# Sara-H-dev/Semantic_Segmentation_Of_StyleGAN2_Artifacts

Hardware: AMD Instinct MI355X
Metric: training images/sec at 1024^2 bs=8 per GPU (MS-UNet Swin-T, fwd+DynamicLoss+bwd+AdamW) (higher is better)
Workload: dtype bf16; 1 GPU; 1xMI355X 1024x1024 bs=8 Swin-T MS-UNet train step; model=MS-UNet swin_t, global_batch=8, world_size=1, img_size=1024, parallelism=dp1, grad_allreduce=f32, dead_branches=executed (no grad), step_execution=eager, params=42881040

## Files before the change

include/msunet_hip.h:

```cpp
#ifndef MSUNET_HIP_H
#define MSUNET_HIP_H

#ifdef __cplusplus
extern "C" {
#endif

int msu_layernorm_fwd(int dtype, int mode, const void* x, const void* b, const float* bscale,
                      long rows_per_sample, void* s_out, const float* gamma, const float* beta,
                      void* y, float* mean, float* rstd, long rows, int C, int H, int W, int Cin,
                      float eps, void* stream);
int msu_layernorm_bwd(int dtype, int mode, const void* dy, const void* x, const void* dres,
                      const float* gamma, const float* mean, const float* rstd, void* dx,
                      void* db, const float* bscale, long rows_per_sample, float* part,
                      int nparts, float* dgamma, float* dbeta, long rows, int C, int H, int W,
                      int Cin, int accumulate, void* stream);
int msu_layernorm_bwd3(int dtype, int mode, const void* dy, const void* x, const void* dres,
                       const void* dres2, const void* dres3, const float* gamma, const float* mean,
                       const float* rstd, void* dx, void* db, const float* bscale, long rows_per_sample,
                       float* part, int nparts, float* dgamma, float* dbeta, long rows, int C, int H, int W,
                       int Cin, int accumulate, void* stream);
int msu_ln_part_blocks(long rows, int C);
int msu_colsum_batch(int nseg, const float* const* part, const long* stride, const int* nparts, const int* n,
                     float* const* out, int accumulate, void* stream);
int msu_tail_reduce_mode(int mode);
// ... 48 lines not shown
                      float* workspace, void* unused, int nchunk, int B, int H, int W, int Cin,
                      int Cout, void* stream);
int msu_conv3x3_wgrad2(int dtype, int in_mode, const void* X, const void* dY, float* dW, float* db,
                       float* workspace, int nchunk, int B, int H, int W, int Cin, int Cout, int accumulate,
                       void* stream);

int msu_win_attn_qkv_supported(int C, int nh);
int msu_win_attn_qkv_fwd(int dtype, const void* x, const void* w_qkv, const float* b_qkv, const float* table,
                         void* out, void* qkv_out, void* keep, float* workspace, int B, int H, int W, int C, int nh,
                         int shift, float p_drop, unsigned long long seed, const unsigned long long* seed_dev,
                         void* stream);
int msu_win_attn_qkv_fwd2(int dtype, const void* x, const void* w_qkv, const float* b_qkv, const float* table,
                          const void* w_proj, const float* b_proj, void* out, void* o_out, void* qkv_out, void* keep,
                          float* workspace, int B, int H, int W, int C, int nh, int shift, float p_drop,
                          unsigned long long seed, const unsigned long long* seed_dev, void* stream);

int msu_wgrad_splits(long M, int N, int K);
long msu_wgrad_workspace(long M, int N, int K);
int msu_linear_wgrad(int dtype, const void* dY, const void* X, float* dW, float* db, float* workspace,
                     long M, int N, int K, int accumulate, void* stream);
int msu_linear_wgrad_ld(int dtype, const void* dY, const void* X, float* dW, long ldw, float* db,
                        float* workspace, long M, int N, int K, int accumulate, void* stream);
int msu_linear_wgrad_plan(int dtype, long M, int N, int K, int* out6);

int msu_linear_bwd_supported(long M, int K, int N);
long msu_linear_bwd_workspace(long M, int K, int N);
int msu_linear_bwd(int dtype, const void* dY, const void* X, const void* Wt, const void* H, void* dX, float* dW,
                   float* db, float* workspace, long M, int K, int N, int accumulate, void* stream);

int msu_tok_gemm_supported(long M, int N, int K);
int msu_tok_gemm_supported_epi(long M, int N, int K, int epi);
int msu_tok_gemm(int dtype, const void* A, const void* A2, int K1, const void* W, const float* bias, void* Y,
                 void* Y2, const void* H, long M, int N, int K, int epi, void* stream);
int msu_tok_gemm_plan(long M, int N, int K, long* out6);
int msu_tok_gemm_plan_epi(long M, int N, int K, int epi, int concat, long* out6);
int msu_nt_gemm_supported(long M, int N, int K);
int msu_nt_gemm_plan(long M, int N);
int msu_nt_gemm_plan2(long M, int N, int K, int epi, int wkn, long* out8);
int msu_nt_gemm_mode(int mode);
int msu_nt_gemm(int dtype, const void* A, const void* W, const float* bias, void* Y, void* Y2, const void* H,
                long M, int N, int K, int epi, void* stream);
int msu_nt_gemm_cat(int dtype, const void* A, const void* A2, int K1, const void* W, const float* bias, void* Y,
                    long M, int N, int K, void* stream);
int msu_nt_gemm_kn(int dtype, const void* A, const void* Wk, const float* bias, void* Y, void* Y2, const void* H,
                   long M, int N, int K, int epi, void* stream);

// ... 82 lines not shown
```

semantic_segmentation_of_stylegan2_artifacts_amd/_lib.py:

```python
import ctypes
import os

from . import switches

_HERE = os.path.dirname(os.path.abspath(__file__))
LIB_PATH = switches.get("MSU_LIB_OVERRIDE") or os.path.join(_HERE, "libmsunet_hip.so")

P = ctypes.c_void_p
I = ctypes.c_int
L = ctypes.c_long
F = ctypes.c_float
D = ctypes.c_double
U64 = ctypes.c_ulonglong

SIGNATURES = {
    "msu_ln_part_blocks": (I, [L, I]),
    "msu_layernorm_fwd": (I, [I, I, P, P, P, L, P, P, P, P, P, P, L, I, I, I, I, F, P]),
    "msu_layernorm_bwd": (I, [I, I, P, P, P, P, P, P, P, P, P, L, P, I, P, P, L, I, I, I, I, I, P]),
    "msu_layernorm_bwd3": (I, [I, I, P, P, P, P, P, P, P, P, P, P, P, L, P, I, P, P, L, I, I, I, I, I, P]),
    "msu_reduce_rows": (I, [P, I, I, L, P, I, P]),
    "msu_tail_reduce_mode": (I, [I]),
    "msu_conv_mode": (I, [I]),
    "msu_conv3x3_route": (I, [I, I, I]),
    "msu_head_fwd": (I, [I, P, P, P, P, P, P, P, L, I, F, P]),
# ... 31 lines not shown
    "msu_grad_sumsq2": (I, [P, L, P, L, P, I, P, P]),
    "msu_grad_clip_scale": (I, [P, I, P, D, P, P, P]),
    "msu_adamw_dev": (I, [P, P, P, P, L, P, D, D, D, D, P, P, P]),
    "msu_adamw_dev2": (I, [P, P, P, P, L, P, D, D, D, D, P, P, P, I, I, P]),
    "msu_adamw_dev3": (I, [P, P, P, P, P, L, P, D, D, D, D, D, P, P, P, I, I, P]),
    "msu_swap_cast": (I, [P, P, P, I, L, P]),
    "msu_step_advance": (I, [P, P, P]),
    "msu_loss_scale_step": (I, [P, P, P, P, P, P, D, D, I, P]),
    "msu_cast": (I, [I, P, P, L, P]),
    "msu_colsum_batch": (I, [I, P, P, P, P, P, I, P]),
    "msu_conv3x3_weight": (I, [I, P, P, I, I, I, P]),
    "msu_transpose16_multi": (I, [P, P, P, I, I, P]),
    "msu_conv3x3_fwd": (I, [I, I, P, P, P, P, I, I, I, I, I, P]),
    "msu_conv3x3_fwd2": (I, [I, I, P, P, P, P, P, I, I, I, I, I, P]),
    "msu_conv3x3_dgrad": (I, [I, I, P, P, P, P, I, I, I, I, I, P]),
    "msu_conv3x3_wgrad_workspace": (L, [I, I, I, I, I]),
    "msu_conv3x3_wgrad": (I, [I, I, P, P, P, P, P, P, I, I, I, I, I, I, P]),
    "msu_conv3x3_wgrad2": (I, [I, I, P, P, P, P, P, I, I, I, I, I, I, I, P]),
    "msu_wgrad_splits": (I, [L, I, I]),
    "msu_wgrad_workspace": (L, [L, I, I]),
    "msu_linear_wgrad": (I, [I, P, P, P, P, P, L, I, I, I, P]),
    "msu_linear_wgrad_ld": (I, [I, P, P, P, L, P, P, L, I, I, I, P]),
    "msu_linear_wgrad_plan": (I, [I, L, I, I, P]),
    "msu_linear_bwd_supported": (I, [L, I, I]),
    "msu_linear_bwd_workspace": (L, [L, I, I]),
    "msu_linear_bwd": (I, [I, P, P, P, P, P, P, P, P, L, I, I, I, P]),
    "msu_tok_gemm_supported": (I, [L, I, I]),
    "msu_tok_gemm_supported_epi": (I, [L, I, I, I]),
    "msu_tok_gemm": (I, [I, P, P, I, P, P, P, P, P, L, I, I, I, P]),
    "msu_tok_gemm_plan": (I, [L, I, I, P]),
    "msu_tok_gemm_plan_epi": (I, [L, I, I, I, I, P]),
    "msu_nt_gemm_supported": (I, [L, I, I]),
    "msu_nt_gemm_plan": (I, [L, I]),
    "msu_nt_gemm_plan2": (I, [L, I, I, I, I, P]),
    "msu_nt_gemm_mode": (I, [I]),
    "msu_nt_gemm": (I, [I, P, P, P, P, P, P, L, I, I, I, P]),
    "msu_nt_gemm_kn": (I, [I, P, P, P, P, P, P, L, I, I, I, P]),
    "msu_nt_gemm_cat": (I, [I, P, P, I, P, P, P, L, I, I, P]),
    "msu_metrics_nblk": (I, [L]),
    "msu_seg_metrics": (I, [I, P, P, I, L, F, P, I, P, P]),
    "msu_augment_batch": (I, [P, P, P, P, P, P, I, I, I, P]),
    "msu_augment_gather": (I, [P, P, P, I, P, P, P, P, I, I, I, P]),
    "msu_pred_maps_nblk": (I, [I, I]),
    "msu_pred_maps": (I, [I, P, P, P, I, I, I, F, F, F, F, I, I, P, P, P, P, P, P, P, P]),
}

# ... 38 lines not shown
```

semantic_segmentation_of_stylegan2_artifacts_amd/csrc/gemm_wgrad.hip:

```cpp
#include <stdlib.h>

#include "common.h"
#include "mfma_frag.h"
#include "reduce.h"

#ifndef MSU_EXP
#define MSU_EXP 0
#endif

namespace {

constexpr int BM = 64;

MSU_DEV void unpack8(const u32x4& q, float (&v)[8]) {
#pragma unroll
  for (int i = 0; i < 4; ++i) {
    v[2 * i] = __uint_as_float(q[i] << 16);
    v[2 * i + 1] = __uint_as_float(q[i] & 0xffff0000u);
  }
}

template <typename T, int NTW>
__global__ void __launch_bounds__(256) wgrad_kernel(const T* __restrict__ dY, const T* __restrict__ X,
                                                    float* __restrict__ part, float* __restrict__ dbpart,
// ... 69 lines not shown
      for (int r = 0; r < BM; ++r) dbacc += to_f32(A[r * LDT + tid]);
    }
    if (more) store_regs(buf ^ 1);
    __syncthreads();
    buf ^= 1;
  }
  float* out = part + (long)blockIdx.y * N * K;
#pragma unroll
  for (int i = 0; i < NTW; ++i)
#pragma unroll
    for (int j = 0; j < NTW; ++j)
#pragma unroll
      for (int r = 0; r < 4; ++r) {
        const int n = n0 + wn + 16 * i + (lane >> 4) * 4 + r;
        const int k = k0 + wk + 16 * j + (lane & 15);
        if (n < N && k < K) out[(long)n * K + k] = acc[i][j][r];
      }
  if (do_bias && tid < BT && n0 + tid < N) dbpart[(long)blockIdx.y * N + n0 + tid] = dbacc;
}

template <int WN, int WK> constexpr int wgrad_nw() { return WN * WK == 3 ? 3 : 4; }

template <typename T, int NTW, int WN, int WK, int NST>
__global__ void __launch_bounds__(256) wgrad_wave_kernel(const bf16_t* __restrict__ dY, const bf16_t* __restrict__ X,
                                                         float* __restrict__ part, float* __restrict__ dbpart,
                                                         long M, int N, int K, long mchunk, int ntiles) {
  constexpr int NW = wgrad_nw<WN, WK>();
  constexpr int WM = NW / (WN * WK), WT = 16 * NTW, BN = WN * WT, BK = WK * WT, RS = 32 * WM;
  static_assert(WM * WN * WK == NW, "wave split");
  constexpr int SA = (BN + 8) / 8, SB = (BK + 8) / 8;
  constexpr int LA = 8 * SA, LB = 8 * SB;
  constexpr int SLOTS = RS * (SA + SB);
  constexpr int INS = ((SLOTS + 63) / 64 + NW - 1) / NW * NW;
  constexpr int PER_WAVE = INS / NW;
  constexpr int STG = INS * 64 * 8;
  static_assert(NST >= 2 && PER_WAVE * (NST - 2) < 64, "vmcnt");
  extern __shared__ __attribute__((aligned(16))) unsigned char smem_raw[];
  bf16_t* lds = reinterpret_cast<bf16_t*>(smem_raw);
  const int tid = threadIdx.x, lane = tid & 63;
  const int wave = __builtin_amdgcn_readfirstlane(tid >> 6);
  const int wni = wave % WN, wki = (wave / WN) % WK, wmi = wave / (WN * WK);
  const int ntk = K / BK;
  const int item = xcd_remap(blockIdx.x, gridDim.x);
  const int split = item / ntiles, tile = item - split * ntiles;
  const int tn = tile / ntk, tk = tile - (tile / ntk) * ntk;
  const int n0 = tn * BN, k0 = tk * BK;
  const long m_begin = (long)split * mchunk;
  long m_end = m_begin + mchunk;
  if (m_end > M) m_end = M;
  const int nstage = m_end > m_begin ? (int)((m_end - m_begin + RS - 1) / RS) : 0;

  int srow[PER_WAVE], soff[PER_WAVE];
  bool sisA[PER_WAVE];
#pragma unroll
  for (int r = 0; r < PER_WAVE; ++r) {
    const int s = 64 * (wave + NW * r) + lane;
    if (s < RS * SA) {
      const int row = s / SA, c = s - (s / SA) * SA;
      srow[r] = row;
      soff[r] = row * N + n0 + (c < SA - 1 ? 8 * c : 0);
      sisA[r] = true;
    } else {
      const int t = s < SLOTS ? s - RS * SA : 0;
      const int row = t / SB, c = t - (t / SB) * SB;
      srow[r] = s < SLOTS ? row : RS;
      soff[r] = row * K + k0 + (c < SB - 1 ? 8 * c : 0);
      sisA[r] = false;
    }
  }
  auto issue = [&](int st) __attribute__((always_inline)) {
    bf16_t* buf = lds + (st % NST) * STG;
    const long m0 = m_begin + (long)st * RS;
    const long rem = m_end - m0;
    const int valid = rem > RS ? RS : (rem < 0 ? 0 : (int)rem);
    const bf16_t* baseA = dY + m0 * N;
    const bf16_t* baseB = X + m0 * K;
#pragma unroll
    for (int r = 0; r < PER_WAVE; ++r) {
      const bf16_t* src = (sisA[r] ? baseA : baseB) + soff[r];
      glds16(srow[r] < valid ? (const void*)src : zero_src(64 * r + lane), buf + 64 * 8 * (wave + NW * r));
    }
  };

  f32x4 acc[NTW][NTW];
  f32x4 accb[NTW];
#pragma unroll
  for (int i = 0; i < NTW; ++i) {
    accb[i] = f32x4{0.f, 0.f, 0.f, 0.f};
#pragma unroll
    for (int j = 0; j < NTW; ++j) acc[i][j] = f32x4{0.f, 0.f, 0.f, 0.f};
  }
  const bool do_bias = dbpart != nullptr && tk == 0 && wki == 0;
  const bf16x8 ones = splat8<T>(1.0f, 1.0f, 1.0f);
  const int q = (lane & 15) >> 2, p4 = 4 * (lane & 3), r0 = wmi * 32 + 2 * (4 * ((lane >> 4) & 1) + q) + (lane >> 5);
  const int laneA = r0 * LA + wni * WT + p4, laneB = RS * LA + r0 * LB + wki * WT + p4;
  auto tr8 = [](const bf16_t* p, int second) {
    typedef __attribute__((address_space(3))) msu_v4s lds_v4s;
    const msu_v4s lo = __builtin_amdgcn_ds_read_tr16_b64_v4i16((lds_v4s*)(p));
    const msu_v4s hi = __builtin_amdgcn_ds_read_tr16_b64_v4i16((lds_v4s*)(p + second));
    msu_v4s both[2] = {lo, hi};
    return *reinterpret_cast<bf16x8*>(both);
  };

#pragma unroll
  for (int st = 0; st < NST - 1; ++st) issue(st);
  for (int st = 0; st < nstage; ++st) {
    wait_vmcnt<PER_WAVE * (NST - 2)>();
    __builtin_amdgcn_s_barrier();
    issue(st + NST - 1);
    if constexpr (MSU_EXP & 2) continue;
    const bf16_t* buf = lds + (st % NST) * STG;
    const uint32_t pa = lds_u32(buf + laneA), pb = lds_u32(buf + laneB);
    bf16x8 bf[NTW], af[2];
    unroll_for<NTW>([&](auto J) {
      constexpr int j = decltype(J)::value;
// ... 44 lines not shown
#pragma unroll
          for (int r = 0; r < 4; ++r) mine[(IH * NTW * 4 + (i - h0) * 4 + r) * 64 + lane] = accb[i][r];
        }
      }
      __syncthreads();
      if (wmi == 0) {
#pragma unroll
        for (int w = 1; w < WM; ++w) {
          const float* other = red + ((long)wnk * (WM - 1) + w - 1) * PW;
#pragma unroll
          for (int i = h0; i < h0 + IH; ++i) {
#pragma unroll
            for (int j = 0; j < NTW; ++j)
#pragma unroll
              for (int r = 0; r < 4; ++r) acc[i][j][r] += other[(((i - h0) * NTW + j) * 4 + r) * 64 + lane];
#pragma unroll
            for (int r = 0; r < 4; ++r) accb[i][r] += other[(IH * NTW * 4 + (i - h0) * 4 + r) * 64 + lane];
          }
        }
      }
    });
  }
  if (wmi != 0) return;
  float* out = part + (long)split * N * K;
#pragma unroll
  for (int i = 0; i < NTW; ++i)
#pragma unroll
    for (int j = 0; j < NTW; ++j)
#pragma unroll
      for (int r = 0; r < 4; ++r) {
        const int n = n0 + wni * WT + 16 * i + (lane >> 4) * 4 + r;
        const int k = k0 + wki * WT + 16 * j + (lane & 15);
        out[(long)n * K + k] = acc[i][j][r];
      }
  if (do_bias && (lane & 15) == 0) {
#pragma unroll
    for (int i = 0; i < NTW; ++i)
#pragma unroll
      for (int r = 0; r < 4; ++r)
        dbpart[(long)split * N + n0 + wni * WT + 16 * i + (lane >> 4) * 4 + r] = accb[i][r];
  }
}

struct WavePlan {
  int ntw = 0, wn = 1, wk = 1, nst = 3, S = 1;
  int slabs() const { return S; }
};

inline void pick_wave_split(int nt, int kt, int& wn, int& wk) {
  static const int cand[8][2] = {{4, 1}, {2, 2}, {1, 4}, {3, 1}, {1, 3}, {2, 1}, {1, 2}, {1, 1}};
  long best = -1;
  for (const auto& c : cand) {
    if (nt % c[0] || kt % c[1]) continue;
    const long cost = (long)nt * kt / c[1] + (long)kt * nt / c[0];
    if (best < 0 || cost < best) {
      best = cost;
      wn = c[0];
      wk = c[1];
    }
  }
}

inline WavePlan wave_plan(long M, int N, int K) {
  WavePlan p;
// ... 64 lines not shown
    launch_wave<T, NTW, WN, WK, 3>(grid, dY, X, part, dbpart, M, N, K, mchunk, ntiles, st);                         \
    return 0;                                                                                                       \
  }
  MSU_WAVE(6, 1, 1) MSU_WAVE(6, 2, 1) MSU_WAVE(6, 4, 1) MSU_WAVE(6, 1, 2) MSU_WAVE(6, 2, 2) MSU_WAVE(6, 1, 4)
  MSU_WAVE(6, 3, 1) MSU_WAVE(6, 1, 3)
  MSU_WAVE(8, 1, 1) MSU_WAVE(8, 2, 1) MSU_WAVE(8, 4, 1) MSU_WAVE(8, 1, 2) MSU_WAVE(8, 2, 2) MSU_WAVE(8, 1, 4)
  MSU_WAVE(8, 3, 1) MSU_WAVE(8, 1, 3)
#undef MSU_WAVE
  return -3;
}

inline int tile_of(int N, int K) { return (N % 128 == 0 && K % 128 == 0) ? 128 : 96; }

inline int pick_splits(long M, int N, int K) {
  const int bt = tile_of(N, K);
  const long tiles = (long)((N + bt - 1) / bt) * ((K + bt - 1) / bt);
  long s = (1024 + tiles - 1) / tiles;
  const long max_s = (M + 511) / 512;
  if (s > max_s) s = max_s;
  if (s < 1) s = 1;
  return (int)s;
}

}

extern "C" {

int msu_wgrad_splits(long M, int N, int K) { return pick_splits(M, N, K); }

long msu_wgrad_workspace(long M, int N, int K) {
  const int S = pick_splits(M, N, K);
  long ws = (long)S * N * K + (long)S * N;
  const WavePlan p = wave_plan(M, N, K);
  if (p.ntw) {
    const long w2 = (long)p.slabs() * N * K + (long)p.slabs() * N;
    if (w2 > ws) ws = w2;
  }
  return ws;
}

int msu_linear_wgrad_ld(int dtype, const void* dY, const void* X, float* dW, long ldw, float* db,
                        float* workspace, long M, int N, int K, int accumulate, void* stream) {
  if (N % 8 || K % 8 || M < 0 || ldw < K) return -2;
  hipStream_t st = (hipStream_t)stream;
  if constexpr ((MSU_EXP & 256) != 0) return 0;
  if (M == 0) {
    if (!accumulate) hipMemset2DAsync(dW, sizeof(float) * ldw, 0, sizeof(float) * K, N, st);
    if (db && !accumulate) hipMemsetAsync(db, 0, sizeof(float) * N, st);
    return MSU_CHECK_LAUNCH();
// ... 54 lines not shown
```

semantic_segmentation_of_stylegan2_artifacts_amd/csrc/reduce.h:

```cpp
#pragma once
#include <mutex>

#include "common.h"

extern int g_msu_tail_on;

namespace {

struct ColSegs {
  const float* part[3];
  float* out[3];
  long n[3];
  long stride[3];
  long rowlen[3], ldo[3];
  int bend[3];
  int nseg;
};

template <int PL, int V>
__global__ void __launch_bounds__(256) colsum_kernel(ColSegs sg, int nparts, int accmask) {
  constexpr int NC = 256 / PL;
  typedef float vec __attribute__((ext_vector_type(V)));
  __shared__ vec red[PL][NC + (V == 1 ? 1 : 0)];
  int seg = 0;
// ... 113 lines not shown
#pragma unroll
      for (int u = 0; u < 4; ++u) v[u] = *reinterpret_cast<const float4*>(part + (long)(q + u * CB_PL) * stride + i);
#pragma unroll
      for (int u = 0; u < 4; ++u) { s.x += v[u].x; s.y += v[u].y; s.z += v[u].z; s.w += v[u].w; }
    }
    for (; q < np; q += CB_PL) {
      const float4 v = *reinterpret_cast<const float4*>(part + (long)q * stride + i);
      s.x += v.x; s.y += v.y; s.z += v.z; s.w += v.w;
    }
  }
  __shared__ float4 red[CB_PL][CB_NC];
  red[ly][lx] = s;
  __syncthreads();
  if (ly == 0 && i < n) {
    float4 t = red[0][lx];
#pragma unroll
    for (int k = 1; k < CB_PL; ++k) { t.x += red[k][lx].x; t.y += red[k][lx].y; t.z += red[k][lx].z; t.w += red[k][lx].w; }
    float4* o = reinterpret_cast<float4*>(cb.out[seg] + i);
    if (cb.accumulate) { const float4 v = *o; t.x += v.x; t.y += v.y; t.z += v.z; t.w += v.w; }
    *o = t;
  }
}

constexpr int TAIL_GS = 32, TAIL_SLOTS = 64, TAIL_WORDS = 2048;
__device__ int g_tail_cnt[TAIL_SLOTS * TAIL_WORDS];

inline int tail_slot(hipStream_t st) {
  static std::mutex mu;
  static hipStream_t owner[TAIL_SLOTS];
  static int used = 0;
  if (!g_msu_tail_on) return -1;
  std::lock_guard<std::mutex> lk(mu);
  for (int i = 0; i < used; ++i)
    if (owner[i] == st) return i;
  if (used == TAIL_SLOTS) return -1;
  owner[used] = st;
  return used++;
}

MSU_DEV void tail_st(float* p, float v) { __hip_atomic_store(p, v, __ATOMIC_RELAXED, __HIP_MEMORY_SCOPE_AGENT); }
MSU_DEV void tail_st4(float* p, float4 v) {
  tail_st(p, v.x);
  tail_st(p + 1, v.y);
  tail_st(p + 2, v.z);
  tail_st(p + 3, v.w);
}
// ... 58 lines not shown
```

semantic_segmentation_of_stylegan2_artifacts_amd/ops.py:

```python
import contextlib
import ctypes
import functools

import torch

from . import _lib, switches

_DT = {torch.float32: 0, torch.bfloat16: 1, torch.float16: 2}
_LOW = (torch.bfloat16, torch.float16)


def _dt(t):
    try:
        return _DT[t.dtype]
    except KeyError:
        raise TypeError(f"unsupported activation dtype {t.dtype} (float32 / bfloat16 / float16)") from None


def _need_cuda(*ts):
    for t in ts:
        if t is not None and not t.is_cuda:
            raise RuntimeError("msunet HIP ops need tensors on a HIP device (no CPU fallback)")


# ... 72 lines not shown

def join_side_streams():
    for idx, st in _side_streams.items():
        torch.cuda.current_stream(idx).wait_stream(st)


def _guard_side_write(p, ev):
    p = getattr(p, "_msu_param", p)
    p._msu_side_event = ev
    _side_event_params.append(p)
    if not getattr(p, "_msu_side_hooked", False):
        def hook(grad, p=p):
            e = getattr(p, "_msu_side_event", None)
            if grad is not None and e is not None:
                torch.cuda.current_stream(p.device).wait_event(e)
            return grad
        p.register_hook(hook)
        p._msu_side_hooked = True


_side_keep = []
_side_event_params = []
_ln_pending = []
_bwd_task = -1
backward_discards = 0


_RES_HANDOFF = switches.on("MSU_RES_HANDOFF")
_res_handoff = {}
_res_closed = set()
_res_keys = iter(range(1, 1 << 62))
res_handoff_calls = 0
res_parked = 0
res_dropped = 0


def residual_handoff_key():
    return next(_res_keys) if (_RES_HANDOFF and torch.is_grad_enabled()) else 0


def _park(key, g):
    global res_parked
    if not key:
        return False
    _join_at_end_of_backward()
    if key in _res_closed:
        return False
    _res_handoff.setdefault(key, []).append(g)
    res_parked += 1
    return True


def _take(key):
    if not key:
        return []
    _join_at_end_of_backward()
    _res_closed.add(key)
    return _res_handoff.pop(key, [])


def reset_backward_state():
    global _bwd_task
    _ln_pending.clear()
    _res_handoff.clear()
    _res_closed.clear()
    _side_keep.clear()
    for p in _side_event_params:
        p._msu_side_event = None
    _side_event_params.clear()
    _bwd_task = -1


def _end_of_backward():
    global res_dropped
    _flush_ln()
    res_dropped += sum(len(v) for v in _res_handoff.values())
    join_side_streams()
    reset_backward_state()


def _join_at_end_of_backward():
    global _bwd_task, backward_discards
    task = torch._C._current_graph_task_id()
    if task == _bwd_task and task != -1:
        return
    if _bwd_task != -1:
        backward_discards += 1
        reset_backward_state()
    torch.autograd.Variable._execution_engine.queue_callback(_end_of_backward)
    _bwd_task = task


@contextlib.contextmanager
def _on_side(device, reads=(), writes=()):
    side = _side_stream_for(device)
    side.wait_stream(torch.cuda.current_stream(device))
    _join_at_end_of_backward()
    for t in reads:
        t.record_stream(side)
        _side_keep.append(t)
    with torch.cuda.stream(side):
        yield
    ev = torch.cuda.Event()
    ev.record(side)
    for p in writes:
        if p is not None:
            _guard_side_write(p, ev)
    _notify(*writes)


def _direct(*params):
    return all(p is not None and getattr(p, "_msu_direct", False) and p.grad is not None for p in params)


def _notify(*params):
    if _grad_ready is not None:
        for p in params:
# ... 338 lines not shown
    ctx.bias_param = qkv_bias if isinstance(qkv_bias, torch.nn.Parameter) else None
    ctx.table_param = table if isinstance(table, torch.nn.Parameter) else None
    ctx.cfg = (num_heads, shift, float(p_drop), seed)


def _attn_backward(ctx, dout, _dkeep, _dws=None):
    qkv, qkv_bias, table, seed_dev, keep = ctx.saved_tensors
    if dout is None:
        return None, None, None, None, None, None, None, None
    kp = _p(keep) if keep.numel() else None
    nh, shift, p_drop, seed = ctx.cfg
    B, H, W, C3 = qkv.shape
    C = C3 // 3
    dout = _as(dout, qkv.dtype)
    need = _attn_bwd_ws(qkv.dtype, B, H, W, C, nh)
    ws = getattr(ctx, "aux_ws", None)
    if ws is not None and _ATTN_AUX and qkv.dtype in _LOW and ws.numel() >= need:
        tbl = None
    else:
        ws = torch.empty(need, device=qkv.device, dtype=torch.float32)
        tbl = _p(table)
    dqkv = torch.empty_like(qkv)
    bp, tp = ctx.bias_param, ctx.table_param
    if bp is not None and tp is not None and _side_enabled and _side_attn_tail and _direct(bp, tp):
        _lib.call("msu_win_attn_bwd2", _dt(qkv), _p(qkv), _p(qkv_bias), tbl, _p(dout), _p(dqkv),
                  None, None, _p(ws), B, H, W, C, nh, shift, p_drop, seed, _p(seed_dev), kp,
                  _s(qkv), -1)
        with _on_side(qkv.device, reads=(ws,), writes=(bp, tp)):
            _lib.call("msu_win_attn_bwd_tail2", _dt(qkv), _p(ws), _p(tp.grad), _p(bp.grad), B, H, W, C, nh, 1,
                      _s(qkv))
        return dqkv, None, None, None, None, None, None, None
    dtable = torch.empty_like(table)
    dbias = torch.empty(3 * C, device=qkv.device, dtype=torch.float32)
    _lib.call("msu_win_attn_bwd", _dt(qkv), _p(qkv), _p(qkv_bias), tbl, _p(dout), _p(dqkv),
              _p(dtable), _p(dbias), _p(ws), B, H, W, C, nh, shift, p_drop, seed, _p(seed_dev), kp, _s(qkv))
    return dqkv, dbias, dtable, None, None, None, None, None


_window_attention = _define(
    "window_attention",
    "(Tensor qkv, Tensor qkv_bias, Tensor table, int num_heads, int shift, float p_drop, int seed, Tensor? seed_dev)"
    " -> (Tensor, Tensor, Tensor)",
    _attn_impl, _attn_fake, _attn_setup, _attn_backward)


def window_attention(qkv, qkv_bias, table, num_heads, shift, p_drop=0.0, seed=0, seed_dev=None):
# ... 193 lines not shown
def _gemm_dx(dy, w, epi=TOK_PLAIN, h=None, param=None):
    N, K = w.shape
    M = dy.numel() // N
    wt = _shadow_t(param, w.dtype)
    if gemm_route(M, K, N, epi) == "nt" and wt is None:
        return nt_gemm_kn(dy, w, epi, h)
    return _gemm(dy, _wt(w) if wt is None else wt, None, epi, h)


def _gelu16(h):
    g = torch.empty_like(h)
    _lib.call("msu_gelu_fwd", _dt(h), _p(h), _p(g), h.numel(), _s(h))
    return g


def _wgrad_launch(dy, x, dw, db, M, N, K, acc, x_gelu_of=None):
    if x is None:
        x = _gelu16(x_gelu_of)
    ws = torch.empty(_lib.lib().msu_wgrad_workspace(M, N, K), device=x.device, dtype=torch.float32)
    _lib.call("msu_linear_wgrad_ld", _dt(x), _p(dy), _p(x), _p(dw), dw.stride(0), _p(db), _p(ws), M, N, K, acc,
              _s(x))


def _wgrad(dy, x, weight, bias, M, N, K, x_gelu_of=None, side_ok=True):
    src = x if x is not None else x_gelu_of
    if not (_direct(weight) and (bias is None or _direct(bias))):
        dw = torch.empty(N, K, device=src.device, dtype=torch.float32)
        db = torch.empty(N, device=src.device, dtype=torch.float32) if bias is not None else None
        _wgrad_launch(dy, x, dw, db, M, N, K, 0, x_gelu_of)
        return dw, db
    side = _side_enabled and _side_wgrad and side_ok
    with _on_side(src.device, (dy, src), (weight, bias)) if side else contextlib.nullcontext():
        _wgrad_launch(dy, x, weight.grad, None if bias is None else bias.grad, M, N, K, 1, x_gelu_of)
    if not side:
        _notify(weight, bias)
    return None, None


def _shadow(param, dt):
    sh = getattr(param, "_msu_shadow", None)
    if sh is not None and sh.dtype == dt and getattr(param, "_msu_shadow_ver", -1) == param._version:
        return sh
    return param.to(dt)


_SHADOW_T = True


def _shadow_t(param, dt):
    if param is None or not _SHADOW_T:
        return None
    sh = getattr(param, "_msu_shadow_t", None)
    if sh is not None and sh.dtype == dt and getattr(param, "_msu_shadow_ver", -1) == param._version:
# ... 73 lines not shown
    return _linear_fwd(x, weight, bias)


def _linear_fake(x, weight, bias, handoff=0):
    return x.new_empty(*x.shape[:-1], weight.shape[0])


def _linear_setup(ctx, inputs, output):
    x, weight, bias = inputs[:3]
    ctx.save_for_backward(x)
    ctx.params = (weight, bias)
    ctx.handoff = inputs[3] if len(inputs) > 3 else 0


_LINBWD = switches.on("MSU_LINBWD")
_LINBWD_MIN_M = 65536


linbwd_calls = 0


def _linbwd(dy, x, weight, bias, M, N, K, h=None, gelu_x=False):
    global linbwd_calls
    if not _LINBWD or x.dtype not in _LOW or M < _LINBWD_MIN_M:
        return None
    if not _direct(weight) or (bias is not None and not _direct(bias)):
        return None
    L = _lib.lib()
    if not L.msu_linear_bwd_supported(M, K, N):
        return None
    wt = _shadow_t(weight, x.dtype)
    if wt is None:
        wt = _wt(_shadow(weight, x.dtype))
    if bias is not None:
        ev = getattr(bias, "_msu_side_event", None)
        if ev is not None:
            torch.cuda.current_stream(x.device).wait_event(ev)
    dx = torch.empty(*dy.shape[:-1], K, device=dy.device, dtype=dy.dtype)
    ws = torch.empty(L.msu_linear_bwd_workspace(M, K, N), device=x.device, dtype=torch.float32)
    _lib.call("msu_linear_bwd", _dt(x), _p(dy), _p(None if gelu_x else x.contiguous()), _p(wt), _p(h), _p(dx),
              _p(weight.grad),
              _p(None if bias is None else bias.grad), _p(ws), M, K, N, 1, _s(x))
    linbwd_calls += 1
    _notify(weight, bias)
    return dx

# ... 71 lines not shown

def _linear_cat_setup(ctx, inputs, output):
    x, skip, weight, bias = inputs[:4]
    ctx.save_for_backward(x, skip)
    ctx.params = (weight, bias)
    ctx.handoff = inputs[4] if len(inputs) > 4 else 0


def _linear_cat_backward(ctx, dy):
    x, skip = ctx.saved_tensors
    weight, bias = ctx.params
    W = _shadow(weight, x.dtype)
    dy = _as(dy, x.dtype)
    N = W.shape[0]
    C1, C2 = x.shape[-1], skip.shape[-1]
    M = dy.numel() // N
    outs = []
    wt = _shadow_t(weight, W.dtype)
    for lo, hi in ((0, C1), (C1, C1 + C2)):
        outs.append(_gemm(dy, W[:, lo:hi].t().contiguous() if wt is None else wt[lo:hi]))
    if _park(ctx.handoff, outs[1]):
        outs[1] = None
    direct = _direct(weight, bias)
    if direct:
        dw, db, acc = weight.grad, bias.grad, 1
    else:
        dw = torch.empty(N, C1 + C2, device=x.device, dtype=torch.float32)
        db = torch.empty(N, device=x.device, dtype=torch.float32)
        acc = 0
    side = direct and _side_enabled and _side_wgrad
    with _on_side(x.device, (dy, x, skip), (weight, bias)) if side else contextlib.nullcontext():
        _wgrad_launch(dy, x, dw[:, :C1], db, M, N, C1, acc)
        _wgrad_launch(dy, skip, dw[:, C1:], None, M, N, C2, acc)
    if not direct:
        return outs[0], outs[1], dw, db, None
    if not side:
        _notify(weight, bias)
    return outs[0], outs[1], None, None, None


_linear_cat = _define("linear_cat", "(Tensor x, Tensor skip, Tensor weight, Tensor bias, int handoff=0) -> Tensor",
                      _linear_cat_impl, _linear_cat_fake, _linear_cat_setup, _linear_cat_backward)


def linear_cat(x, skip, weight, bias, handoff=0):
    _need_cuda(x)
    dt = act_dtype()
    x, skip = _as(x, dt), _as(skip, dt)
    N, K = weight.shape
    C1, C2 = x.shape[-1], skip.shape[-1]
    M = x.numel() // C1
    if dt in _LOW and bias is not None and C1 + C2 == K and _cat_route(M, N, K, C1) is not None:
# ... 755 lines not shown
```

semantic_segmentation_of_stylegan2_artifacts_amd/switches.py:

```python
import os
import warnings

SWITCHES = {
    "MSU_LIB_OVERRIDE": ("", "path of another libmsunet_hip.so (tools/build_exp.sh ablation builds)",
                         "DESIGN 4c"),
    "MSU_WGRAD_SIDE": ("1", "0: every weight gradient on the main stream (determinism bisection)",
                       "DESIGN 4b, 7 (side stream +1.6 %)"),
    "MSU_ATTN_QKV": ("1", "0: the unfused stage-0 qkv Linear + window attention + proj (C = 96 and C = 128)",
                     "DESIGN 4d (r04c: +0.8 % on Swin-T), 7 round 10 (r10a: +0.6 % on Swin-B)"),
    "MSU_GEMM_ROUTE": ("", "force a GEMM route: lib (hipBLASLt) / tok / nt",
                       "DESIGN 7 (r03c: hand-written +2.7 % over hipBLASLt)"),
    "MSU_NT_PP": ("0", "1: the ping-pong NT GEMM (gemm_pp.h) where it tiles exactly, else the persistent one",
                  "DESIGN 7 (r05g: 0.72-0.98x of the persistent kernel; no-store ablation 1.07-1.66x)"),
    "MSU_LINBWD": ("1", "0: stage-0 Linear backward as input-gradient GEMM + side-stream weight gradient",
                   "DESIGN 7 (r03af: one-pass +1.4 %)"),
    "MSU_CONV_SIDE": ("1", "0: the refine-conv weight gradients on the main stream",
                      "DESIGN 7 (r04s: side +0.2 %)"),
    "MSU_TAIL": ("1", "0: LayerNorm parameter-gradient partials summed by a colsum launch, not in the kernel",
                 "DESIGN 7 (r05i: +0.5 %, host -4 ms/step)"),
    "MSU_ATTN_AUX": ("1", "0: each attention backward rebuilds its relative-bias image instead of reusing the "
                     "forward's workspace", "DESIGN 7 (r05az)"),
    "MSU_MLP_INFER": ("1", "0: no-grad stage-0 MLPs on the token-GEMM pair instead of the fused kernel",
                      "DESIGN 7 (r05am: +1.3 %)"),
    "MSU_MLP_LN": ("1", "0: no-grad stage-0 blocks run norm2's residual-add LayerNorm as its own kernel before the "
                   "fused MLP", "DESIGN 7 (r05at)"),
    "MSU_MLP_TRAIN": ("1", "0: training stage-0 MLPs on the token-GEMM pair (H and GELU(H) stored) instead of "
                      "the fused kernel storing H only", "DESIGN 7 (r05ao)"),
    "MSU_LN_DEFER": ("1", "0: each LayerNorm backward sums its parameter-gradient partials itself (in-kernel "
                     "tail) instead of one batched reduction per width", "DESIGN 7 (r06)"),
    "MSU_CONV_DYN": ("1", "0: the refine-conv kernel's static tile schedule (blockIdx.x + k * gridDim.x) instead "
# ... 39 lines not shown
```

Before: 182.0 images/s.

## Group Linear weight-gradient GEMMs of a Swin block into one launch

Parks each Linear weight-gradient GEMM with the same token count instead of launching it right away, then runs the parked set as one grouped wave kernel with a shared split-M plan. A batched column-sum kernel reduces the partials. Parked work is flushed at stage changes, before side-stream writes to the same parameters, and at the end of backward. The aim is fewer small launches and better CU fill than separate per-layer wgrad kernels. The cost is extra bookkeeping and ordering hazards, and grads computed later, which may reduce overlap with the main stream.

```diff
diff --git a/include/msunet_hip.h b/include/msunet_hip.h
--- a/include/msunet_hip.h
+++ b/include/msunet_hip.h
@@ -94,6 +94,11 @@
 int msu_linear_wgrad_ld(int dtype, const void* dY, const void* X, float* dW, long ldw, float* db,
                         float* workspace, long M, int N, int K, int accumulate, void* stream);
 int msu_linear_wgrad_plan(int dtype, long M, int N, int K, int* out6);
+int msu_linear_wgrad_group(int dtype, int np, const void* const* dY, const void* const* X, float* const* dW,
+                           const long* ldw, float* const* db, float* workspace, const long* M, const int* N,
+                           const int* K, int accumulate, void* stream);
+long msu_wgrad_group_workspace(int dtype, int np, const long* M, const int* N, const int* K);
+int msu_linear_wgrad_group_plan(int dtype, int np, const long* M, const int* N, const int* K, long* out);
 
 int msu_linear_bwd_supported(long M, int K, int N);
 long msu_linear_bwd_workspace(long M, int K, int N);
diff --git a/semantic_segmentation_of_stylegan2_artifacts_amd/_lib.py b/semantic_segmentation_of_stylegan2_artifacts_amd/_lib.py
--- a/semantic_segmentation_of_stylegan2_artifacts_amd/_lib.py
+++ b/semantic_segmentation_of_stylegan2_artifacts_amd/_lib.py
@@ -77,6 +77,9 @@
     "msu_linear_wgrad": (I, [I, P, P, P, P, P, L, I, I, I, P]),
     "msu_linear_wgrad_ld": (I, [I, P, P, P, L, P, P, L, I, I, I, P]),
     "msu_linear_wgrad_plan": (I, [I, L, I, I, P]),
+    "msu_linear_wgrad_group": (I, [I, I, P, P, P, P, P, P, P, P, P, I, P]),
+    "msu_wgrad_group_workspace": (L, [I, I, P, P, P]),
+    "msu_linear_wgrad_group_plan": (I, [I, I, P, P, P, P]),
     "msu_linear_bwd_supported": (I, [L, I, I]),
     "msu_linear_bwd_workspace": (L, [L, I, I]),
     "msu_linear_bwd": (I, [I, P, P, P, P, P, P, P, P, L, I, I, I, P]),
diff --git a/semantic_segmentation_of_stylegan2_artifacts_amd/csrc/gemm_wgrad.hip b/semantic_segmentation_of_stylegan2_artifacts_amd/csrc/gemm_wgrad.hip
--- a/semantic_segmentation_of_stylegan2_artifacts_amd/csrc/gemm_wgrad.hip
+++ b/semantic_segmentation_of_stylegan2_artifacts_amd/csrc/gemm_wgrad.hip
@@ -115,9 +115,9 @@
 template <int WN, int WK> constexpr int wgrad_nw() { return WN * WK == 3 ? 3 : 4; }
 
 template <typename T, int NTW, int WN, int WK, int NST>
-__global__ void __launch_bounds__(256) wgrad_wave_kernel(const bf16_t* __restrict__ dY, const bf16_t* __restrict__ X,
-                                                         float* __restrict__ part, float* __restrict__ dbpart,
-                                                         long M, int N, int K, long mchunk, int ntiles) {
+MSU_DEV void wgrad_wave_body(const bf16_t* __restrict__ dY, const bf16_t* __restrict__ X, float* __restrict__ out,
+                             long ldo, float* __restrict__ dbout, int accumulate, long m_begin, long m_end, int N,
+                             int K, int tile) {
   constexpr int NW = wgrad_nw<WN, WK>();
   constexpr int WM = NW / (WN * WK), WT = 16 * NTW, BN = WN * WT, BK = WK * WT, RS = 32 * WM;
   static_assert(WM * WN * WK == NW, "wave split");
@@ -134,13 +134,8 @@
   const int wave = __builtin_amdgcn_readfirstlane(tid >> 6);
   const int wni = wave % WN, wki = (wave / WN) % WK, wmi = wave / (WN * WK);
   const int ntk = K / BK;
-  const int item = xcd_remap(blockIdx.x, gridDim.x);
-  const int split = item / ntiles, tile = item - split * ntiles;
   const int tn = tile / ntk, tk = tile - (tile / ntk) * ntk;
   const int n0 = tn * BN, k0 = tk * BK;
-  const long m_begin = (long)split * mchunk;
-  long m_end = m_begin + mchunk;
-  if (m_end > M) m_end = M;
   const int nstage = m_end > m_begin ? (int)((m_end - m_begin + RS - 1) / RS) : 0;
 
   int srow[PER_WAVE], soff[PER_WAVE];
@@ -183,7 +178,7 @@
 #pragma unroll
     for (int j = 0; j < NTW; ++j) acc[i][j] = f32x4{0.f, 0.f, 0.f, 0.f};
   }
-  const bool do_bias = dbpart != nullptr && tk == 0 && wki == 0;
+  const bool do_bias = dbout != nullptr && tk == 0 && wki == 0;
   const bf16x8 ones = splat8<T>(1.0f, 1.0f, 1.0f);
   const int q = (lane & 15) >> 2, p4 = 4 * (lane & 3), r0 = wmi * 32 + 2 * (4 * ((lane >> 4) & 1) + q) + (lane >> 5);
   const int laneA = r0 * LA + wni * WT + p4, laneB = RS * LA + r0 * LB + wki * WT + p4;
@@ -274,7 +269,6 @@
     });
   }
   if (wmi != 0) return;
-  float* out = part + (long)split * N * K;
 #pragma unroll
   for (int i = 0; i < NTW; ++i)
 #pragma unroll
@@ -283,15 +277,64 @@
       for (int r = 0; r < 4; ++r) {
         const int n = n0 + wni * WT + 16 * i + (lane >> 4) * 4 + r;
         const int k = k0 + wki * WT + 16 * j + (lane & 15);
-        out[(long)n * K + k] = acc[i][j][r];
+        float* o = out + (long)n * ldo + k;
+        *o = accumulate ? *o + acc[i][j][r] : acc[i][j][r];
       }
   if (do_bias && (lane & 15) == 0) {
 #pragma unroll
     for (int i = 0; i < NTW; ++i)
 #pragma unroll
-      for (int r = 0; r < 4; ++r)
-        dbpart[(long)split * N + n0 + wni * WT + 16 * i + (lane >> 4) * 4 + r] = accb[i][r];
-  }
+      for (int r = 0; r < 4; ++r) {
+        float* o = dbout + n0 + wni * WT + 16 * i + (lane >> 4) * 4 + r;
+        *o = accumulate ? *o + accb[i][r] : accb[i][r];
+      }
+  }
+}
+
+template <typename T, int NTW, int WN, int WK, int NST>
+__global__ void __launch_bounds__(256) wgrad_wave_kernel(const bf16_t* __restrict__ dY, const bf16_t* __restrict__ X,
+                                                         float* __restrict__ part, float* __restrict__ dbpart,
+                                                         long M, int N, int K, long mchunk, int ntiles) {
+  const int item = xcd_remap(blockIdx.x, gridDim.x);
+  const int split = item / ntiles, tile = item - split * ntiles;
+  const long m_begin = (long)split * mchunk;
+  long m_end = m_begin + mchunk;
+  if (m_end > M) m_end = M;
+  wgrad_wave_body<T, NTW, WN, WK, NST>(dY, X, part + (long)split * N * K, K, dbpart ? dbpart + (long)split * N : nullptr,
+                                       0, m_begin, m_end, N, K, tile);
+}
+
+constexpr int WG_MAX = 16;
+struct WgradGroup {
+  const bf16_t* dY[WG_MAX];
+  const bf16_t* X[WG_MAX];
+  float* out[WG_MAX];
+  float* dbo[WG_MAX];
+  long M[WG_MAX];
+  long ldo[WG_MAX];
+  int N[WG_MAX], K[WG_MAX];
+  int tiles[WG_MAX];
+  int end[WG_MAX];
+  long rows;
+  int np, accumulate;
+};
+
+template <typename T, int NTW, int NST>
+__global__ void __launch_bounds__(256) wgrad_wave_group_kernel(WgradGroup g) {
+  const int item = xcd_remap(blockIdx.x, gridDim.x);
+  int p = 0;
+  while (p + 1 < g.np && item >= g.end[p]) ++p;
+  const int local = item - (p == 0 ? 0 : g.end[p - 1]);
+  const int ntiles = g.tiles[p];
+  const int split = local / ntiles, tile = local - split * ntiles;
+  const long M = g.M[p];
+  const int N = g.N[p], K = g.K[p];
+  const long m_begin = (long)split * g.rows;
+  long m_end = m_begin + g.rows;
+  if (m_end > M) m_end = M;
+  float* dbo = g.dbo[p];
+  wgrad_wave_body<T, NTW, 2, 2, NST>(g.dY[p], g.X[p], g.out[p] + (long)split * N * K, g.ldo[p],
+                                     dbo ? dbo + (long)split * N : nullptr, g.accumulate, m_begin, m_end, N, K, tile);
 }
 
 struct WavePlan {
@@ -402,9 +445,165 @@
   return (int)s;
 }
 
+struct GroupPlan {
+  int ntw = 0;
+  long R = 0, items = 0;
+  bool direct = false;
+  int S[WG_MAX], tiles[WG_MAX];
+};
+
+inline long group_items(int np, const long* M, const int* tiles, long R, int* S) {
+  long items = 0;
+  for (int p = 0; p < np; ++p) {
+    const long s = M[p] > 0 ? (M[p] + R - 1) / R : 1;
+    if (S) S[p] = (int)s;
+    items += s * tiles[p];
+  }
+  return items;
+}
+
+inline bool group_plan(int dtype, int np, const long* M, const int* N, const int* K, GroupPlan& gp) {
+  if (!msu_is16(dtype) || np < 1 || np > WG_MAX) return false;
+  bool t96 = true, t128 = true;
+  long maxM = 0;
+  for (int p = 0; p < np; ++p) {
+    if (M[p] < 0 || N[p] <= 0 || K[p] <= 0 || (long)N[p] * K[p] > 0x7fffffffL) return false;
+    t96 = t96 && N[p] % 192 == 0 && K[p] % 192 == 0;
+    t128 = t128 && N[p] % 256 == 0 && K[p] % 256 == 0;
+    if (M[p] > maxM) maxM = M[p];
+  }
+  if (!t96 && !t128) return false;
+  gp.ntw = t96 ? 6 : 8;
+  const int bt = 32 * gp.ntw;
+  for (int p = 0; p < np; ++p) gp.tiles[p] = (N[p] / bt) * (K[p] / bt);
+  long lo = 8, hi = (maxM + 31) / 32;
+  if (hi < lo) hi = lo;
+  if (group_items(np, M, gp.tiles, 32 * hi, nullptr) <= 256) {
+    while (lo < hi) {
+      const long mid = (lo + hi) / 2;
+      if (group_items(np, M, gp.tiles, 32 * mid, nullptr) <= 256) hi = mid;
+      else lo = mid + 1;
+    }
+  }
+  gp.R = 32 * hi;
+  gp.items = group_items(np, M, gp.tiles, gp.R, gp.S);
+  if (gp.items > 0x7fffffffL) return false;
+  gp.direct = true;
+  for (int p = 0; p < np; ++p) gp.direct = gp.direct && gp.S[p] == 1;
+  return true;
+}
+
+inline long group_workspace(const GroupPlan& gp, int np, const int* N, const int* K) {
+  if (gp.direct) return 0;
+  long ws = 0;
+  for (int p = 0; p < np; ++p) ws += (long)gp.S[p] * ((long)N[p] * K[p] + N[p]);
+  return ws;
+}
+
+template <typename T, int NTW>
+void launch_wave_group(const WgradGroup& g, int items, hipStream_t st) {
+  constexpr int WT = 16 * NTW, SLOTS = 32 * 2 * ((2 * WT + 8) / 8), INS = ((SLOTS + 63) / 64 + 3) / 4 * 4;
+  constexpr size_t lds = (size_t)3 * INS * 64 * 16;
+  static_assert(lds <= 160 * 1024, "ring");
+  auto kern = wgrad_wave_group_kernel<T, NTW, 3>;
+  static bool attr_set = false;
+  if (!attr_set) {
+    (void)hipFuncSetAttribute((const void*)kern, hipFuncAttributeMaxDynamicSharedMemorySize, (int)lds);
+    attr_set = true;
+  }
+  hipLaunchKernelGGL(kern, dim3((unsigned)items), dim3(256), lds, st, g);
+}
+
 }
 
 extern "C" {
+
+int msu_linear_wgrad_group_plan(int dtype, int np, const long* M, const int* N, const int* K, long* out) {
+  GroupPlan gp;
+  if (!group_plan(dtype, np, M, N, K, gp)) return 1;
+  out[0] = 16 * gp.ntw;
+  out[1] = gp.R;
+  out[2] = gp.items;
+  out[3] = gp.direct ? 1 : 0;
+  for (int p = 0; p < np; ++p) out[4 + p] = gp.S[p];
+  return 0;
+}
+
+long msu_wgrad_group_workspace(int dtype, int np, const long* M, const int* N, const int* K) {
+  GroupPlan gp;
+  if (!group_plan(dtype, np, M, N, K, gp)) return -1;
+  return group_workspace(gp, np, N, K);
+}
+
+int msu_linear_wgrad_group(int dtype, int np, const void* const* dY, const void* const* X, float* const* dW,
+                           const long* ldw, float* const* db, float* workspace, const long* M, const int* N,
+                           const int* K, int accumulate, void* stream) {
+  hipStream_t st = (hipStream_t)stream;
+  if constexpr ((MSU_EXP & 256) != 0) return 0;
+  GroupPlan gp;
+  if (!group_plan(dtype, np, M, N, K, gp)) return 1;
+  for (int p = 0; p < np; ++p) {
+    if (ldw[p] < K[p]) return -2;
+    if (!gp.direct && (ldw[p] % 4 || ((uintptr_t)dW[p] & 15) || ((uintptr_t)db[p] & 15))) return 1;
+  }
+  if (!gp.direct && (workspace == nullptr || ((uintptr_t)workspace & 15))) return -2;
+  WgradGroup g{};
+  ColGroup cg{};
+  float* w = workspace;
+  int end = 0, blocks = 0, nseg = 0;
+  for (int p = 0; p < np; ++p) {
+    const long nk = (long)N[p] * K[p];
+    g.dY[p] = (const bf16_t*)dY[p];
+    g.X[p] = (const bf16_t*)X[p];
+    g.M[p] = M[p];
+    g.N[p] = N[p];
+    g.K[p] = K[p];
+    g.tiles[p] = gp.tiles[p];
+    end += gp.tiles[p] * gp.S[p];
+    g.end[p] = end;
+    if (gp.direct) {
+      g.out[p] = dW[p];
+      g.dbo[p] = db[p];
+      g.ldo[p] = ldw[p];
+      continue;
+    }
+    g.out[p] = w;
+    g.ldo[p] = K[p];
+    w += gp.S[p] * nk;
+    g.dbo[p] = db[p] ? w : nullptr;
+    w += (long)gp.S[p] * N[p];
+    cg.part[nseg] = g.out[p];
+    cg.out[nseg] = dW[p];
+    cg.n[nseg] = (int)nk;
+    cg.nparts[nseg] = gp.S[p];
+    cg.rowlen[nseg] = K[p];
+    cg.ldo[nseg] = ldw[p];
+    cg.bend[nseg++] = blocks += colgroup_blocks(nk);
+    if (db[p]) {
+      cg.part[nseg] = g.dbo[p];
+      cg.out[nseg] = db[p];
+      cg.n[nseg] = N[p];
+      cg.nparts[nseg] = gp.S[p];
+      cg.rowlen[nseg] = N[p];
+      cg.ldo[nseg] = N[p];
+      cg.bend[nseg++] = blocks += colgroup_blocks(N[p]);
+    }
+  }
+  g.rows = gp.R;
+  g.np = np;
+  g.accumulate = gp.direct ? (accumulate != 0) : 0;
+  if (gp.ntw == 6) {
+    MSU_DISPATCH16(dtype, T, (launch_wave_group<T, 6>(g, (int)gp.items, st)));
+  } else {
+    MSU_DISPATCH16(dtype, T, (launch_wave_group<T, 8>(g, (int)gp.items, st)));
+  }
+  if (!gp.direct) {
+    cg.nseg = nseg;
+    cg.accumulate = accumulate != 0;
+    hipLaunchKernelGGL(colsum_group_kernel, dim3(blocks), dim3(256), 0, st, cg);
+  }
+  return MSU_CHECK_LAUNCH();
+}
 
 int msu_wgrad_splits(long M, int N, int K) { return pick_splits(M, N, K); }
 
diff --git a/semantic_segmentation_of_stylegan2_artifacts_amd/csrc/reduce.h b/semantic_segmentation_of_stylegan2_artifacts_amd/csrc/reduce.h
--- a/semantic_segmentation_of_stylegan2_artifacts_amd/csrc/reduce.h
+++ b/semantic_segmentation_of_stylegan2_artifacts_amd/csrc/reduce.h
@@ -159,6 +159,52 @@
   }
 }
 
+constexpr int CG_MAX = 32, CG_PL = 8, CG_NC = 32;
+struct ColGroup {
+  const float* part[CG_MAX];
+  float* out[CG_MAX];
+  int n[CG_MAX];
+  int nparts[CG_MAX];
+  int rowlen[CG_MAX];
+  long ldo[CG_MAX];
+  int bend[CG_MAX];
+  int nseg;
+  int accumulate;
+};
+
+inline int colgroup_blocks(long n) { return (int)((n / 4 + CG_NC - 1) / CG_NC); }
+
+__global__ void __launch_bounds__(256) colsum_group_kernel(ColGroup cg) {
+  int seg = 0;
+  while (seg + 1 < cg.nseg && (int)blockIdx.x >= cg.bend[seg]) ++seg;
+  const int b0 = seg == 0 ? 0 : cg.bend[seg - 1];
+  const float* __restrict__ part = cg.part[seg];
+  const int n = cg.n[seg], np = cg.nparts[seg];
+  const int lx = threadIdx.x % CG_NC, ly = threadIdx.x / CG_NC;
+  const int i = (((int)blockIdx.x - b0) * CG_NC + lx) * 4;
+  float4 s = {0.f, 0.f, 0.f, 0.f};
+  if (i < n) {
+#pragma unroll 4
+    for (int q = ly; q < np; q += CG_PL) {
+      const float4 v = *reinterpret_cast<const float4*>(part + (long)q * n + i);
+      s.x += v.x; s.y += v.y; s.z += v.z; s.w += v.w;
+    }
+  }
+  __shared__ float4 red[CG_PL][CG_NC];
+  red[ly][lx] = s;
+  __syncthreads();
+  if (ly == 0 && i < n) {
+    float4 t = red[0][lx];
+#pragma unroll
+    for (int k = 1; k < CG_PL; ++k) { t.x += red[k][lx].x; t.y += red[k][lx].y; t.z += red[k][lx].z; t.w += red[k][lx].w; }
+    const int rl = cg.rowlen[seg];
+    const long oi = (long)(i / rl) * cg.ldo[seg] + (i - (i / rl) * rl);
+    float4* o = reinterpret_cast<float4*>(cg.out[seg] + oi);
+    if (cg.accumulate) { const float4 v = *o; t.x += v.x; t.y += v.y; t.z += v.z; t.w += v.w; }
+    *o = t;
+  }
+}
+
 constexpr int TAIL_GS = 32, TAIL_SLOTS = 64, TAIL_WORDS = 2048;
 __device__ int g_tail_cnt[TAIL_SLOTS * TAIL_WORDS];
 
diff --git a/semantic_segmentation_of_stylegan2_artifacts_amd/ops.py b/semantic_segmentation_of_stylegan2_artifacts_amd/ops.py
--- a/semantic_segmentation_of_stylegan2_artifacts_amd/ops.py
+++ b/semantic_segmentation_of_stylegan2_artifacts_amd/ops.py
@@ -118,6 +118,7 @@
 _side_keep = []
 _side_event_params = []
 _ln_pending = []
+_wgrad_pending = []
 _bwd_task = -1
 backward_discards = 0
 
@@ -158,6 +159,7 @@
 def reset_backward_state():
     global _bwd_task
     _ln_pending.clear()
+    _wgrad_pending.clear()
     _res_handoff.clear()
     _res_closed.clear()
     _side_keep.clear()
@@ -170,6 +172,7 @@
 def _end_of_backward():
     global res_dropped
     _flush_ln()
+    _flush_wgrad()
     res_dropped += sum(len(v) for v in _res_handoff.values())
     join_side_streams()
     reset_backward_state()
@@ -189,6 +192,7 @@
 
 @contextlib.contextmanager
 def _on_side(device, reads=(), writes=()):
+    _flush_wgrad_of(writes)
     side = _side_stream_for(device)
     side.wait_stream(torch.cuda.current_stream(device))
     _join_at_end_of_backward()
@@ -573,6 +577,7 @@
         tbl = _p(table)
     dqkv = torch.empty_like(qkv)
     bp, tp = ctx.bias_param, ctx.table_param
+    _flush_wgrad_of((bp, tp))
     if bp is not None and tp is not None and _side_enabled and _side_attn_tail and _direct(bp, tp):
         _lib.call("msu_win_attn_bwd2", _dt(qkv), _p(qkv), _p(qkv_bias), tbl, _p(dout), _p(dqkv),
                   None, None, _p(ws), B, H, W, C, nh, shift, p_drop, seed, _p(seed_dev), kp,
@@ -812,6 +817,101 @@
               _s(x))
 
 
+_WGRAD_GROUP = switches.on("MSU_WGRAD_GROUP")
+_WGRAD_GROUP_MAX = 16
+_WGRAD_GROUP_BYTES = 0
+wgrad_groups = 0
+wgrad_parked = 0
+
+
+def _wgrad_tile(dt, N, K):
+    if dt not in _LOW:
+        return 0
+    return 96 if (N % 192 == 0 and K % 192 == 0) else (128 if (N % 256 == 0 and K % 256 == 0) else 0)
+
+
+def _wgrad_held_bytes(e):
+    return 2 * e[5] * (e[6] + e[7])
+
+
+def _wgrad_park(dy, x, x_gelu_of, weight, bias, M, N, K, dw, db):
+    global wgrad_parked
+    src = x if x is not None else x_gelu_of
+    tile = _wgrad_tile(src.dtype, N, K) if _WGRAD_GROUP else 0
+    if not tile or dy.dtype != src.dtype:
+        return False
+    _join_at_end_of_backward()
+    entry = (dy, x, x_gelu_of, weight, bias, M, N, K, dw, db)
+    if _wgrad_pending:
+        f = _wgrad_pending[0]
+        fsrc = f[1] if f[1] is not None else f[2]
+        outs = {o.data_ptr() for e in _wgrad_pending for o in e[8:10] if o is not None}
+        if (f[5] != M or _wgrad_tile(fsrc.dtype, f[6], f[7]) != tile or fsrc.dtype != src.dtype
+                or fsrc.device != src.device or len(_wgrad_pending) >= _WGRAD_GROUP_MAX
+                or dw.data_ptr() in outs or (db is not None and db.data_ptr() in outs)
+                or (_WGRAD_GROUP_BYTES and sum(map(_wgrad_held_bytes, _wgrad_pending)) + _wgrad_held_bytes(entry)
+                    > _WGRAD_GROUP_BYTES)):
+            _flush_wgrad()
+    _wgrad_pending.append(entry)
+    wgrad_parked += 1
+    return True
+
+
+def _wgrad_group_launch(group):
+    L = _lib.lib()
+    k = len(group)
+    xs = [e[1] if e[1] is not None else _gelu16(e[2]) for e in group]
+    Ms = (ctypes.c_long * k)(*[e[5] for e in group])
+    Ns = (ctypes.c_int * k)(*[e[6] for e in group])
+    Ks = (ctypes.c_int * k)(*[e[7] for e in group])
+    dt = _dt(xs[0])
+    n = L.msu_wgrad_group_workspace(dt, k, Ms, Ns, Ks)
+    rc = 1
+    if n >= 0:
+        ws = torch.empty(n, device=xs[0].device, dtype=torch.float32) if n else None
+        P = ctypes.c_void_p * k
+        rc = L.msu_linear_wgrad_group(
+            dt, k, P(*[_p(e[0]) for e in group]), P(*[_p(x) for x in xs]), P(*[_p(e[8]) for e in group]),
+            (ctypes.c_long * k)(*[e[8].stride(0) for e in group]), P(*[_p(e[9]) for e in group]), _p(ws), Ms, Ns, Ks,
+            1, _s(xs[0]))
+        if rc < 0:
+            raise _lib.HipLibraryError(f"msu_linear_wgrad_group failed with code {rc}")
+    if rc:
+        for e, x in zip(group, xs):
+            _wgrad_launch(e[0], x, e[8], e[9], e[5], e[6], e[7], 1)
+
+
+def _flush_wgrad():
+    global wgrad_groups
+    if not _wgrad_pending:
+        return
+    group = list(_wgrad_pending)
+    _wgrad_pending.clear()
+    reads, writes = [], []
+    for e in group:
+        reads += [e[0], e[1] if e[1] is not None else e[2]]
+        writes += [p for p in e[3:5] if p is not None and not any(p is q for q in writes)]
+    side = _side_enabled and _side_wgrad
+    with _on_side(reads[0].device, reads, writes) if side else contextlib.nullcontext():
+        _wgrad_group_launch(group)
+    wgrad_groups += 1
+    if not side:
+        _notify(*writes)
+
+
+def _wgrad_stage(M):
+    if _wgrad_pending and _wgrad_pending[0][5] != M:
+        _flush_wgrad()
+
+
+def _flush_wgrad_of(params):
+    if not _wgrad_pending:
+        return
+    own = [getattr(p, "_msu_param", p) for p in params if p is not None]
+    if any(getattr(q, "_msu_param", q) is p for e in _wgrad_pending for q in e[3:5] if q is not None for p in own):
+        _flush_wgrad()
+
+
 def _wgrad(dy, x, weight, bias, M, N, K, x_gelu_of=None, side_ok=True):
     src = x if x is not None else x_gelu_of
     if not (_direct(weight) and (bias is None or _direct(bias))):
@@ -819,6 +919,10 @@
         db = torch.empty(N, device=src.device, dtype=torch.float32) if bias is not None else None
         _wgrad_launch(dy, x, dw, db, M, N, K, 0, x_gelu_of)
         return dw, db
+    _wgrad_stage(M)
+    if side_ok and _wgrad_park(dy, x, x_gelu_of, weight, bias, M, N, K, weight.grad,
+                               None if bias is None else bias.grad):
+        return None, None
     side = _side_enabled and _side_wgrad and side_ok
     with _on_side(src.device, (dy, src), (weight, bias)) if side else contextlib.nullcontext():
         _wgrad_launch(dy, x, weight.grad, None if bias is None else bias.grad, M, N, K, 1, x_gelu_of)
@@ -938,6 +1042,7 @@
 
 def _linbwd(dy, x, weight, bias, M, N, K, h=None, gelu_x=False):
     global linbwd_calls
+    _wgrad_stage(M)
     if not _LINBWD or x.dtype not in _LOW or M < _LINBWD_MIN_M:
         return None
     if not _direct(weight) or (bias is not None and not _direct(bias)):
@@ -1055,12 +1160,18 @@
     if _park(ctx.handoff, outs[1]):
         outs[1] = None
     direct = _direct(weight, bias)
+    _wgrad_stage(M)
     if direct:
         dw, db, acc = weight.grad, bias.grad, 1
     else:
         dw = torch.empty(N, C1 + C2, device=x.device, dtype=torch.float32)
         db = torch.empty(N, device=x.device, dtype=torch.float32)
         acc = 0
+    if direct and _wgrad_tile(x.dtype, N, C1) and _wgrad_tile(x.dtype, N, C1) == _wgrad_tile(skip.dtype, N, C2):
+        parked = (_wgrad_park(dy, x, None, weight, bias, M, N, C1, dw[:, :C1], db)
+                  and _wgrad_park(dy, skip, None, weight, None, M, N, C2, dw[:, C1:], None))
+        if parked:
+            return outs[0], outs[1], None, None, None
     side = direct and _side_enabled and _side_wgrad
     with _on_side(x.device, (dy, x, skip), (weight, bias)) if side else contextlib.nullcontext():
         _wgrad_launch(dy, x, dw[:, :C1], db, M, N, C1, acc)
diff --git a/semantic_segmentation_of_stylegan2_artifacts_amd/switches.py b/semantic_segmentation_of_stylegan2_artifacts_amd/switches.py
--- a/semantic_segmentation_of_stylegan2_artifacts_amd/switches.py
+++ b/semantic_segmentation_of_stylegan2_artifacts_amd/switches.py
@@ -6,6 +6,8 @@
                          "DESIGN 4c"),
     "MSU_WGRAD_SIDE": ("1", "0: every weight gradient on the main stream (determinism bisection)",
                        "DESIGN 4b, 7 (side stream +1.6 %)"),
+    "MSU_WGRAD_GROUP": ("1", "0: every Linear weight gradient in a launch of its own instead of one grouped launch "
+                        "per Swin block", "DESIGN 4, 4b, 7 (r20a)"),
     "MSU_ATTN_QKV": ("1", "0: the unfused stage-0 qkv Linear + window attention + proj (C = 96 and C = 128)",
                      "DESIGN 4d (r04c: +0.8 % on Swin-T), 7 round 10 (r10a: +0.6 % on Swin-B)"),
     "MSU_GEMM_ROUTE": ("", "force a GEMM route: lib (hipBLASLt) / tok / nt",
```

After: 182.5 images/s, median of 6. No clear change (+0.2%).
